# danielajisafe/A-NeRF

Hardware: AMD Instinct MI355X
Metric: rays/sec at 512×512×128 samples, 24-joint, 8×256 MLP; 1/2/4/8 GPU (higher is better)
Workload: dtype fp32-accurate split fp16: hidden and view layers after exact power-of-two scaling, x = x0+x1 and W = W0+W1 (remainders within 2^-23 of |x|, |W|), the four fp16 MFMA products x_i W_j (dropped: the remainders' ~2^-22 of |x W|, the bound of bf16x6's dropped terms), fp32 accumulate; the bone-direction a

## Files before the change

### a-nerf_amd/build.py

```python
import hashlib
import os
import subprocess
import sys
from concurrent.futures import ThreadPoolExecutor

HERE = os.path.dirname(os.path.abspath(__file__))
CSRC = os.path.join(HERE, "csrc")
HEADER = os.path.join(os.path.dirname(HERE), "include", "anerf.h")
SRC = [os.path.join(CSRC, "anerf_render.hip"), os.path.join(CSRC, "anerf_gemm.hip"),
       os.path.join(CSRC, "anerf_iso.hip"), os.path.join(CSRC, "anerf_mesh.hip"),
       os.path.join(CSRC, "anerf_raster.hip")]
SCAN_HEADER = os.path.join(CSRC, "anerf_scan.hpp")
OUT = os.path.join(HERE, "libanerf_hip.so")
STAMP = OUT + ".stamp"
OBJS = os.path.join(HERE, ".objs")
HIPCC = os.environ.get("HIPCC", "/opt/rocm/bin/hipcc")
FLAGS = ["--offload-arch=gfx950", "-O3", "-std=c++17", "-ffp-contract=off", "-fno-slp-vectorize", "-fPIC", "-shared",
         "-Wno-unused-result"]
CFLAGS = [f for f in FLAGS if f != "-shared"]


def _hash(files, extra=""):
    h = hashlib.sha256()
    h.update((" ".join(FLAGS) + extra).encode())
    for d in files:
        if os.path.isfile(d):
            h.update(os.path.basename(d).encode())
            with open(d, "rb") as f:
                h.update(f.read())
    return h.hexdigest()


def source_hash():
    deps = sorted(os.path.join(CSRC, f) for f in os.listdir(CSRC))
    deps.append(HEADER)
    return _hash(deps)


def unit_deps(src):
    name = os.path.basename(src)
    if name == "anerf_gemm.hip":
        return [src, HEADER]
    if name in ("anerf_mesh.hip", "anerf_raster.hip"):
        return [src, SCAN_HEADER, HEADER]
    if name == "anerf_iso.hip":
        return [src, os.path.join(CSRC, "anerf_iso_table.inc"), SCAN_HEADER, HEADER]
    return [src] + sorted(os.path.join(CSRC, f) for f in os.listdir(CSRC)
                          if f.endswith(".hpp") and f != os.path.basename(SCAN_HEADER)) + [HEADER]


def stamp_matches():
    if not (os.path.exists(OUT) and os.path.exists(STAMP)):
        return False
    with open(STAMP) as f:
        return f.read().strip() == source_hash()


def _object(src, verbose, force=False):
    digest = _hash(unit_deps(src), "-c")
    name = os.path.splitext(os.path.basename(src))[0]
    obj = os.path.join(OBJS, f"{name}.{digest[:20]}.o")
    if os.path.exists(obj) and not force:
        return obj
    tmp = obj + ".tmp"
    cmd = [HIPCC] + CFLAGS + ["-c", "-o", tmp, src]
    if verbose:
        print(" ".join(cmd), file=sys.stderr)
    subprocess.run(cmd, check=True)
    if _hash(unit_deps(src), "-c") != digest:
        os.remove(tmp)
        raise RuntimeError(f"sources of {name} changed during the build: the object was discarded, build again")
    for old in os.listdir(OBJS):
        if old.startswith(name + ".") and old.endswith(".o"):
            os.remove(os.path.join(OBJS, old))
    os.replace(tmp, obj)
    return obj


def build(force=False, verbose=True):
    if not force and stamp_matches():
        return OUT
    digest = source_hash()
    os.makedirs(OBJS, exist_ok=True)
    with ThreadPoolExecutor(max(1, len(SRC))) as ex:
        objs = list(ex.map(lambda s: _object(s, verbose, force), SRC))
    tmp = OUT + ".tmp"
    if os.path.exists(tmp):
        os.remove(tmp)
    cmd = [HIPCC] + FLAGS + ["-o", tmp] + objs
    if verbose:
        print(" ".join(cmd), file=sys.stderr)
    subprocess.run(cmd, check=True)
    if source_hash() != digest:
        if os.path.exists(tmp):
            os.remove(tmp)
        raise RuntimeError("sources changed during the build: the library was discarded, build again")
    os.replace(tmp, OUT)
    with open(STAMP, "w") as f:
        f.write(digest + "\n")
    return OUT


if __name__ == "__main__":
    build(force="--force" in sys.argv)
```

### a-nerf_amd/csrc/anerf_kernels.hpp

```cpp
#pragma once

template <int W, int MR, int PREC>
__device__ __forceinline__ void render_item(const ModelDev& M, const RenderArgs& A, const LdsPlan& P,
                                            float* __restrict__ lds, int64_t ray0) {
    constexpr int WH = W / 2;
    const int tid = threadIdx.x, lane = tid & 63, wave = tid >> 6;
    const int R = A.R, S = A.S, I = A.I, T = S + I;
    const int nr = (int)min((int64_t)R, A.n - ray0);

    for (int r = tid; r < nr; r += blockDim.x) {
        const int64_t i = ray0 + r;
        const float* src = A.rb + i * A.stride;
        float* d = lds + P.ray + 16 * r;
        for (int c = 0; c < 6; ++c) d[c] = src[c];
        d[6] = A.cams ? A.cams[i] : -1.0f;
        d[7] = A.near[i];
        d[8] = A.far[i];
        d[9] = norm3(src[3], src[4], src[5]);
        d[10] = __int_as_float(A.ray_pose ? A.ray_pose[i] : 0);
    }
    __syncthreads();
    for (int idx = tid; idx < nr * M.nj * 12; idx += blockDim.x) {
        const int r = idx / (M.nj * 12), e = idx % (M.nj * 12);
        const int j = e / 12, c = e % 12;
// ... 358 lines not shown
        const float px = A.pts[3 * s], py = A.pts[3 * s + 1], pz = A.pts[3 * s + 2];
        const float* dp = A.dirs + s * A.dir_stride;
        const float dx = dp[0], dy = dp[1], dz = dp[2];
        f32x16 acc[RB], h[RB];
        JointMask mask;
        Ring ring;
        int es = 0;
        const bool pre = mlp_trunk<W, MR, true, PREC>(M, net, lds + P.sk, lds + P.cut, px, py, pz, lane, lds + P.bias, uf,
                                                      wvp, acc, h, ring, mask,
                                                      PREC >= 3 ? net.wviewh : (PREC == 2 ? net.wview6 : net.wview), st,
                                                      es);
        float sig = 0.0f;
        f32x16 av[RBV];
        if constexpr (PREC >= 3) {
            const int es_h = es;
            mlp_layer_h3<RBV, RB, false, true, PREC == 4 ? 4 : 3>(av, acc, h, nullptr, net.wviewh, lane, ring, pre, nullptr,
                                                                  lds + P.bias + (M.D + 1) * W, sig, es, net.ew_view,
                                                                  M.h3_top);
            sig *= pow2f(-es_h);
        } else if constexpr (PREC == 2)
            mlp_layer_x6<RBV, RB, false, true>(av, acc, h, nullptr, net.wview6, lane, ring, pre, nullptr,
                                               lds + P.bias + (M.D + 1) * W, sig);
        else
            mlp_layer<RBV, RB, true, false, true>(av, acc, h, nullptr, net.wview, lane, ring, nullptr,
                                                  lds + P.bias + (M.D + 1) * W, sig);
        sig += __shfl_xor(sig, 32);
        sig += net.balpha;
        const float bs = PREC >= 3 ? pow2f(es) : 1.0f;
        if (M.mrv == 0) view_dir_points<RBV, 0>(av, M, net, lds + P.sk, wvp, lds + P.g, dx, dy, dz, lane, bs);
        else view_dir_points<RBV, 4>(av, M, net, lds + P.sk, wvp, lds + P.g, dx, dy, dz, lane, bs);
        float rgb[3];
#pragma unroll
        for (int c = 0; c < 3; ++c) {
            const float* wr = net.wrgb + (c * 2 + hh) * RBV * 16;
            float a = 0.0f;
#pragma unroll
            for (int rb = 0; rb < RBV; ++rb)
#pragma unroll
                for (int i = 0; i < 16; ++i) a += wr[rb * 16 + i] * relu_act(av[rb][i]);
            a += __shfl_xor(a, 32);
            if constexpr (PREC >= 3) a *= pow2f(-es);
            rgb[c] = a + net.brgb[c];
        }
        if (own && hh == 0 && s_out < A.n) {
            float* o = A.out + 4 * s_out;
            o[0] = rgb[0];
            o[1] = rgb[1];
            o[2] = rgb[2];
            o[3] = sig;
        }
    }
}

__global__ void near_far_given_kernel(const float* __restrict__ rb, int stride, int64_t n, float* __restrict__ near_out,
                                      float* __restrict__ far_out) {
    const int64_t i = (int64_t)blockIdx.x * blockDim.x + threadIdx.x;
    if (i >= n) return;
    near_out[i] = rb[i * stride + 6];
    far_out[i] = rb[i * stride + 7];
}

__global__ void near_far_kernel(const float* __restrict__ rb, int stride, int64_t n, const float* __restrict__ cyls,
                                const int32_t* __restrict__ ray_pose, int n_poses, float* __restrict__ near_out,
                                float* __restrict__ far_out, uint8_t* __restrict__ qnan) {
    const int64_t i = (int64_t)blockIdx.x * blockDim.x + threadIdx.x;
    if (i >= n) return;
    const float* r = rb + i * stride;
    const int pose = ray_pose ? ray_pose[i] : 0;
    if (pose < 0 || pose >= n_poses) {
        near_out[i] = far_out[i] = __int_as_float(0x7fc00000);
        qnan[i] = 1;
        return;
    }
    const float* cy = cyls + 5 * pose;
    const float nearv = r[6], farv = r[7];
    const float rn0 = r[0] + r[3] * nearv, rn1 = r[2] + r[5] * nearv;
    const float rf0 = r[0] + r[3] * farv, rf1 = r[2] + r[5] * farv;
    const float nc0 = cy[0] - rn0, nc1 = cy[1] - rn1;
    const float nf0 = rf0 - rn0, nf1 = rf1 - rn1;
    const float nfn = norm2(nf0, nf1);
    const float scale = norm2(r[3], r[5]);
    const float cross = nc0 * nf1 - nc1 * nf0;
    const float dist = fabsf(cross) / nfn;
    const float rad = cy[2];
    const float Q = sqrtf(rad * rad - dist * dist);
    const float K = (nc0 * nf0 + nc1 * nf1) / nfn;
    const float mask = (Q < K) ? 1.0f : 0.0f;
    near_out[i] = nearv + (mask * (K - Q)) / scale;
    far_out[i] = nearv + (K + Q) / scale;
    qnan[i] = (Q != Q) ? 1 : 0;
}

constexpr int NF_LEAVES = 1024;
constexpr int NF_LDS = 8192;

__global__ void nan_fill_kernel(const float* __restrict__ rb, int stride, int64_t n, int chunk,
                                float* __restrict__ near_io, float* __restrict__ far_io,
                                const uint8_t* __restrict__ qnan, float* __restrict__ scratch) {
    const int64_t c0 = (int64_t)blockIdx.x * chunk;
    const int64_t c1 = min(c0 + chunk, n);
    const int64_t m = c1 - c0;
    __shared__ int any, n_leaves, valid[2];
    __shared__ float means[2];
    __shared__ int leaf_off[NF_LEAVES], leaf_cnt[NF_LEAVES];
    __shared__ float leaf_sum[NF_LEAVES];
    if (threadIdx.x == 0) { any = 0; valid[0] = valid[1] = 0; }
    __syncthreads();
    for (int64_t i = c0 + threadIdx.x; i < c1; i += blockDim.x)
        if (near_io[i] != near_io[i]) any = 1;
    __syncthreads();
    if (!any) return;
    __shared__ int st_a[64], st_b[64];
    __shared__ float st_v[64];
    if (threadIdx.x == 0) n_leaves = np_pairwise_leaves(m, leaf_off, leaf_cnt, NF_LEAVES, st_a, st_b);
    __shared__ float lbuf[NF_LDS];
    float* buf = m <= NF_LDS ? lbuf : scratch + c0;
    for (int v = 0; v < 2; ++v) {
        const float* src = v == 0 ? near_io : far_io;
        int mine = 0;
        for (int64_t i = c0 + threadIdx.x; i < c1; i += blockDim.x) {
            const float x = src[i];
            buf[i - c0] = (x != x) ? 0.0f : x;
            mine += (x == x);
        }
        atomicAdd(&valid[v], mine);
        __syncthreads();
        if (n_leaves >= 0)
            for (int k = threadIdx.x; k < n_leaves; k += blockDim.x) leaf_sum[k] = np_leaf_sum(buf + leaf_off[k], leaf_cnt[k]);
        __syncthreads();
        if (threadIdx.x == 0) {
            const float sum = n_leaves >= 0 ? np_pairwise_combine(leaf_sum, m, st_a, st_b, st_v) : np_pairwise_sum(buf, m);
            means[v] = valid[v] ? (float)((double)sum / (double)valid[v]) : __int_as_float(0x7fc00000);
        }
        __syncthreads();
    }
    for (int64_t i = c0 + threadIdx.x; i < c1; i += blockDim.x) {
        if (qnan[i]) {
            const float* r = rb + i * stride;
            near_io[i] = (means[0] != means[0]) ? r[6] : means[0];
            far_io[i] = (means[1] != means[1]) ? r[7] : means[1];
        }
    }
}

struct PixelSet {
    const int64_t* idx;
    int64_t x0, y0, bw;
    __device__ __forceinline__ int64_t pixel(int64_t t, int W) const {
        return idx ? idx[t] : (y0 + t / bw) * W + x0 + t % bw;
    }
};

__global__ void gen_rays_kernel(const float* __restrict__ c2w, int H, int W, float fx, float fy, float cx, float cy,
                                PixelSet px, int64_t n, float nearv, float farv, float* __restrict__ out) {
    const int64_t t = (int64_t)blockIdx.x * blockDim.x + threadIdx.x;
    if (t >= n) return;
    const int64_t p = px.pixel(t, W);
    const float x = (float)(p % W), y = (float)(p / W);
    const float d0 = (x - cx) / fx;
    const float d1 = -(y - cy) / fy;
    const float d2 = -1.0f;
    float* o = out + t * 11;
    float dd[3];
    for (int r = 0; r < 3; ++r) {
        dd[r] = (d0 * c2w[4 * r + 0] + d1 * c2w[4 * r + 1]) + d2 * c2w[4 * r + 2];
        o[r] = c2w[4 * r + 3];
        o[3 + r] = dd[r];
    }
    o[6] = nearv;
    o[7] = farv;
    const float nn = norm3(dd[0], dd[1], dd[2]);
    o[8] = dd[0] / nn;
    o[9] = dd[1] / nn;
    o[10] = dd[2] / nn;
}

__global__ void compose_fill_kernel(const float* __restrict__ bg, int white, int64_t hw, float* __restrict__ out_rgb,
                                    float* __restrict__ out_disp, float* __restrict__ out_acc) {
    const int64_t p = (int64_t)blockIdx.x * blockDim.x + threadIdx.x;
    if (p >= hw) return;
    for (int c = 0; c < 3; ++c) out_rgb[3 * p + c] = bg ? bg[3 * p + c] : (white ? 1.0f : 0.0f);
    out_disp[p] = 0.0f;
    if (out_acc) out_acc[p] = 0.0f;
}

__global__ void compose_scatter_kernel(const float* __restrict__ rgb, const float* __restrict__ disp,
                                       const float* __restrict__ acc, PixelSet px, int W, int64_t n,
                                       float* __restrict__ out_rgb, float* __restrict__ out_disp,
                                       float* __restrict__ out_acc) {
    const int64_t i = (int64_t)blockIdx.x * blockDim.x + threadIdx.x;
    if (i >= n) return;
    const int64_t p = px.pixel(i, W);
    const float a = acc[i];
    for (int c = 0; c < 3; ++c) out_rgb[3 * p + c] = rgb[3 * i + c] + (1.0f - a) * out_rgb[3 * p + c];
    const float d = disp[i];
    out_disp[p] = (d != d) ? 0.0f : d;
    if (out_acc) out_acc[p] = a;
}

__device__ void encode_row(const ModelDev& M, const float* __restrict__ skts, float px, float py, float pz, float dx,
                           float dy, float dz, float* __restrict__ f) {
    const int nj = M.nj, nv = 1 + 2 * M.mr;
    const int cx = nj * nv + 3 * nj;
    for (int j = 0; j < nj; ++j) {
        float S[12];
        for (int r = 0; r < 3; ++r)
            for (int c = 0; c < 4; ++c) S[4 * r + c] = skts[j * 16 + 4 * r + c];
        float qx, qy, qz;
        joint_local(S, px, py, pz, qx, qy, qz);
        const float dist = norm3(qx, qy, qz);
        const float dn = fmaxf(dist, 1e-12f);
        const float w = M.use_cutoff ? cutoff_w(M.tau, dist, M.cutoff[j]) : 1.0f;
        float u, uf;
        kp_inputs(M.cut_to, M.shift_in, dist, M.cutoff[j], u, uf);
        f[j] = (M.use_cutoff && M.cutoff_inputs) ? u * w : u;
        for (int fi = 0; fi < M.mr; ++fi) {
            float s, c;
            sincosf(uf * (float)(1 << fi), &s, &c);
            f[(1 + 2 * fi) * nj + j] = s * w;
            f[(2 + 2 * fi) * nj + j] = c * w;
        }
        const float wb = M.bone_cut ? cutoff_w(M.tau_b, dist, M.cutoff_b[j]) : 1.0f;
        f[nj * nv + 3 * j + 0] = M.bone_cut ? (qx / dn) * wb : qx / dn;
        f[nj * nv + 3 * j + 1] = M.bone_cut ? (qy / dn) * wb : qy / dn;
        f[nj * nv + 3 * j + 2] = M.bone_cut ? (qz / dn) * wb : qz / dn;
        float ex, ey, ez;
        joint_rot(S, dx, dy, dz, ex, ey, ez);
        const float en = M.view_raw ? 1.0f : fmaxf(norm3(ex, ey, ez), 1e-12f);
        const float e[3] = {ex / en, ey / en, ez / en};
        const float wv = M.cutoff_viewdir ? cutoff_w(M.tau_v, dist, M.cutoff_v[j]) : 1.0f;
        for (int c = 0; c < 3; ++c) {
            f[cx + 3 * j + c] = (M.cutoff_viewdir && M.cutoff_inputs) ? e[c] * wv : e[c];
            for (int fi = 0; fi < M.mrv; ++fi) {
                float s, co;
                sincosf(e[c] * (float)(1 << fi), &s, &co);
                f[cx + (1 + 2 * fi) * 3 * nj + 3 * j + c] = s * wv;
                f[cx + (2 + 2 * fi) * 3 * nj + 3 * j + c] = co * wv;
            }
        }
    }
}

__global__ void encode_points_kernel(ModelDev M, const float* __restrict__ skts, const float* __restrict__ pts,
                                     const float* __restrict__ dirs, int64_t n, float* __restrict__ feat) {
    const int64_t i = (int64_t)blockIdx.x * blockDim.x + threadIdx.x;
    if (i >= n) return;
    const int F = M.nj * (1 + 2 * M.mr) + 3 * M.nj + 3 * M.nj * (1 + 2 * M.mrv);
    encode_row(M, skts, pts[3 * i], pts[3 * i + 1], pts[3 * i + 2], dirs[3 * i], dirs[3 * i + 1], dirs[3 * i + 2],
               feat + i * F);
}
```

### a-nerf_amd/csrc/anerf_mlp.hpp

```cpp
#pragma once

__device__ __forceinline__ __amdgpu_buffer_rsrc_t make_rsrc(const float* p) {
    return __builtin_amdgcn_make_buffer_rsrc((void*)p, 0, 0x7fffffff, 0x00020000);
}
__device__ __forceinline__ f32x2 bload2(__amdgpu_buffer_rsrc_t rs, int voff, int soff) {
    return __builtin_bit_cast(f32x2, __builtin_amdgcn_raw_buffer_load_b64(rs, voff, soff, 0));
}
__device__ __forceinline__ f32x4 bload4(__amdgpu_buffer_rsrc_t rs, int voff, int soff) {
    return __builtin_bit_cast(f32x4, __builtin_amdgcn_raw_buffer_load_b128(rs, voff, soff, 0));
}

template <int RB>
__device__ __forceinline__ void load_bias(f32x16 (&acc)[RB], const float* __restrict__ bp_lds, int hh) {
#pragma unroll
    for (int rb = 0; rb < RB; ++rb) {
        const f32x4* p = reinterpret_cast<const f32x4*>(bp_lds + (rb * 2 + hh) * 16);
        f32x4 v0 = p[0], v1 = p[1], v2 = p[2], v3 = p[3];
        acc[rb] = f32x16{v0[0], v0[1], v0[2], v0[3], v1[0], v1[1], v1[2], v1[3],
                         v2[0], v2[1], v2[2], v2[3], v3[0], v3[1], v3[2], v3[3]};
    }
}

struct Ring {
    float v[4][16];
// ... 283 lines not shown
    for (int g = 0; g < NQ; ++g) {
        __builtin_amdgcn_sched_barrier(0);
        prefetch(g);
        if constexpr (!std::is_same<Side, NoSide>::value) (*side)(g);
        const int ob = g >> 1, s = g & 1;
        out[ob] = mfma_x6(ring.v[g % 4], T[s], out[ob]);
        if (ob == 0) alpha(0, s);
        if (ob + 1 < RBI && (ob + 1 < RBO || ob == 0)) convert_half(ob + 1, s);
        if (RBI > 1) {
#pragma unroll
            for (int p = 0; p < 8; ++p)
                if (pair_group(p, QL) == (g < QL ? -1 : g) || (g == NQ - 1 && pair_group(p, QL) > g))
                    split3_block_pair(h[1], Tn, p);
        }
        x6_group_schedule();
    }
#pragma clang loop unroll(full)
    for (int ib = 1; ib < RBI; ++ib) {
        T[0] = Tn[0];
        T[1] = Tn[1];
        const bool conv_next = ib + 1 < RBI && ib + 1 >= (RBO > 2 ? RBO : 2);
        const int q0 = conv_next ? (NQ > 2 ? 2 : NQ) : 0;
#pragma clang loop unroll(full)
        for (int q = 0; q < NQ; ++q) {
            const int s = q / RBO, ob = q % RBO;
            const int g = NQ + (ib - 1) * NQ + q;
            __builtin_amdgcn_sched_barrier(0);
            prefetch(g);
            if constexpr (!std::is_same<Side, NoSide>::value) (*side)(g);
            out[ob] = mfma_x6(ring.v[g % 4], T[s], out[ob]);
            if (ob == RBO - 1) alpha(ib, s);
            if (ib + 1 < RBI) {
                if (conv_next && q < 2) convert_half(ib + 1, q);
#pragma unroll
                for (int p = 0; p < 8; ++p)
                    if (pair_group(p, q0) == q || (q == NQ - 1 && pair_group(p, q0) > q))
                        split3_block_pair(h[ib + 1], Tn, p);
            }
            x6_group_schedule();
        }
    }
}

typedef _Float16 f16x8 __attribute__((ext_vector_type(8)));
struct H3T {
    unsigned d[2][4];
    __device__ __forceinline__ f16x8 frag(int c) const {
        return __builtin_bit_cast(f16x8, u32x4{d[c][0], d[c][1], d[c][2], d[c][3]});
    }
};

__device__ __forceinline__ float pow2f(int e) { return __builtin_bit_cast(float, (e + 127) << 23); }

__device__ __forceinline__ void split2_pair(float a, float b, float t, H3T& T, int q) {
    typedef _Float16 f16x2 __attribute__((ext_vector_type(2)));
    const float xa = a * t, xb = b * t;
    const unsigned hi = __builtin_bit_cast(unsigned, __builtin_convertvector((f32x2{xa, xb}), f16x2));
    float la, lb;
    asm("v_fma_mix_f32 %0, %1, -1.0, %2 op_sel_hi:[1,0,0]" : "=v"(la) : "v"(hi), "v"(xa));
    asm("v_fma_mix_f32 %0, %1, -1.0, %2 op_sel:[1,0,0] op_sel_hi:[1,0,0]" : "=v"(lb) : "v"(hi), "v"(xb));
    T.d[0][q] = hi;
    T.d[1][q] = __builtin_bit_cast(unsigned, __builtin_convertvector((f32x2{la, lb}), f16x2));
}

__device__ __forceinline__ void split2_block_pair(const f32x16& hb, float t, H3T (&T)[2], int p) {
    const int s = p >> 2, q = p & 3;
    split2_pair(hb[8 * s + 2 * q], hb[8 * s + 2 * q + 1], t, T[s], q);
}

constexpr int H3_NLG = 2;
constexpr int H3_LEAD_IL = 4;
template <int NP, int NV = H3_IL>
__device__ __forceinline__ void h3_group_schedule() {
    group_schedule<NP, H3_NLG, 4 / H3_NLG, NV>();
}

__device__ __forceinline__ f32x16 mfma_f16_32x32x16(f16x8 a, f16x8 b, f32x16 c) {
    return __builtin_amdgcn_mfma_f32_32x32x16_f16(a, b, c, 0, 0, 0);
}

template <int NP>
__device__ __forceinline__ f32x16 mfma_h3(const float (&w)[16], int half, const H3T& x, f32x16 c) {
    const int o = 8 * half;
    const f16x8 w0 = __builtin_bit_cast(f16x8, f32x4{w[o], w[o + 1], w[o + 2], w[o + 3]});
    const f16x8 w1 = __builtin_bit_cast(f16x8, f32x4{w[o + 4], w[o + 5], w[o + 6], w[o + 7]});
    if constexpr (NP == 4) c = mfma_f16_32x32x16(w1, x.frag(1), c);
    c = mfma_f16_32x32x16(w1, x.frag(0), c);
    c = mfma_f16_32x32x16(w0, x.frag(1), c);
    return mfma_f16_32x32x16(w0, x.frag(0), c);
}

template <int RBI>
__device__ __forceinline__ float h3_scale(const f32x16 (&a)[RBI], int& es, int ew, int top, int cap = 60) {
    int m = 0;
#pragma unroll
    for (int rb = 0; rb < RBI; ++rb)
#pragma unroll
        for (int i = 0; i < 16; ++i) {
            const float v = a[rb][i];
            m = max(m, __builtin_bit_cast(int, v));
        }
    m = max(m, __shfl_xor(m, 32));
    int shift = m > 0 ? top - (m >> 23) : 0;
    shift = max(shift, -100 - es - ew);
    shift = min(shift, cap - es - ew);
    shift = min(max(shift, -126), 126);
    es += shift + ew;
    return pow2f(shift);
}

template <int RBO, int RBI, bool OUT_SAME, bool ALPHA, int NP = 3>
__device__ __forceinline__ void mlp_layer_h3(f32x16 (&out)[RBO], f32x16 (&ain)[RBI], f32x16 (&h)[RBI],
                                             const float* __restrict__ bias, const float* __restrict__ wp, int lane,
                                             Ring& ring, bool preloaded, const float* __restrict__ next,
                                             const float* __restrict__ wa, float& sig, int& es, int ew, int top,
                                             int cap = 60) {
    static_assert(RBO <= RBI, "h3 layer shape");
    constexpr int NG = 2 * RBO * RBI;
    constexpr int NS = NG / 2;
    constexpr int PS = 2;
    constexpr int NQ = 2 * RBO;
    const int hh = lane >> 5;
    const __amdgpu_buffer_rsrc_t rs = make_rsrc(wp);
    const __amdgpu_buffer_rsrc_t rn = make_rsrc(next ? next : wp);
    const float t = h3_scale<RBI>(ain, es, ew, top, cap);
    const float S = pow2f(es);
    auto convert_half = [&](int rb, int half) {
#pragma unroll
        for (int i = 8 * half; i < 8 * half + 8; ++i) h[rb][i] = relu_act(ain[rb][i]);
        if (OUT_SAME && rb < RBO) {
            const f32x4* p = reinterpret_cast<const f32x4*>(bias + (rb * 2 + hh) * 16 + 8 * half);
            const f32x4 v0 = p[0], v1 = p[1];
#pragma unroll
            for (int e = 0; e < 4; ++e) {
                out[rb][8 * half + e] = v0[e] * S;
                out[rb][8 * half + 4 + e] = v1[e] * S;
            }
        }
    };
    auto alpha = [&](int ib, int s) {
        if constexpr (ALPHA) {
            const f32x4* w4 = reinterpret_cast<const f32x4*>(wa + hh * 16 * RBI + 16 * ib + 8 * s);
            const f32x4 u0 = w4[0], u1 = w4[1];
#pragma unroll
            for (int j = 0; j < 8; ++j) sig = fmaf(j < 4 ? u0[j] : u1[j - 4], h[ib][8 * s + j], sig);
        }
    };
    if constexpr (!OUT_SAME) {
#pragma unroll
        for (int rb = 0; rb < RBO; ++rb) out[rb] = f32x16{0};
    }
    const bool has_next = next != nullptr;
    auto prefetch = [&](int g) {
        if (g & 1) return;
        const int G = g >> 1;
        if (G + PS < NS)
            load_group<16>(ring.v[(G + PS) % 4], rs, lane, G + PS);
        else if (NS % 4 == 0)
            load_group<16>(ring.v[(G + PS) % 4], rn, lane, has_next ? G + PS - NS : NS - 1);
    };
    auto pair_group = [](int p, int q0) { return q0 + (p * (NQ - q0 > 0 ? NQ - q0 : 1)) / 8; };
    if (!preloaded) {
#pragma unroll
        for (int G = 0; G < PS && G < NS; ++G) load_group<16>(ring.v[G], rs, lane, G);
    }
    convert_half(0, 0);
    convert_half(0, 1);
    H3T T[2], Tn[2];
#pragma unroll
    for (int p = 0; p < 8; ++p) split2_block_pair(h[0], t, T, p);
    constexpr int QL = NQ > 2 ? 2 : NQ;
#pragma clang loop unroll(full)
    for (int g = 0; g < NQ; ++g) {
        __builtin_amdgcn_sched_barrier(0);
        prefetch(g);
        const int ob = g >> 1, s = g & 1;
        out[ob] = mfma_h3<NP>(ring.v[(g >> 1) % 4], g & 1, T[s], out[ob]);
        if (ob == 0) alpha(0, s);
        if (ob + 1 < RBI && (ob + 1 < RBO || ob == 0)) convert_half(ob + 1, s);
        if (RBI > 1) {
#pragma unroll
            for (int p = 0; p < 8; ++p)
                if (pair_group(p, QL) == (g < QL ? -1 : g) || (g == NQ - 1 && pair_group(p, QL) > g))
                    split2_block_pair(h[1], t, Tn, p);
// ... 823 lines not shown
                if constexpr (UX6) u_part_x6<RB>(acc, M, net.wskipu6, uf, lane, ring, P == 2, xs);
            } else if (uf)
                u_part_lds<RB>(acc, M, net.wskipu, uf, lane, ring, after, xs);
            else
                u_part<RB, false>(acc, M, net.wskipu, sk, cut, px, py, pz, lane, nullptr, nullptr, nullptr, ring, after,
                                  st, xs);
            if constexpr (VX6)
                v_part_x6<RB, MR>(acc, M, net.wskipv6, sk, cut, px, py, pz, lane, mask, ring, xs);
            else
                v_part<RB, MR>(acc, M, net.wskipv, sk, cut, px, py, pz, lane, mask, st, xs);
            STAMP(st, 12);
        }
    }
    return pre6;
}

template <int W, int MR, int P>
__device__ void mlp_block(const ModelDev& M, const NetDev& net, const float* __restrict__ ray,
                          const float* __restrict__ sk, const float* __restrict__ cut, const float* __restrict__ z,
                          int n, int s0,
                          const float* __restrict__ G, float* __restrict__ raw_out, int lane,
                          unsigned long long* mfma_count, const float* __restrict__ bias, float* __restrict__ uf,
                          float* __restrict__ wvp, Stamps& st, bool store = true) {
    constexpr int RB = W / 32;
    constexpr int RBV = (W / 2) / 32;
    const int sl = lane & 31, hh = lane >> 5;
    int s = s0 + sl;
    if (s >= n) s = n - 1;
    const float zs = z[s];
    const float px = ray[0] + ray[3] * zs;
    const float py = ray[1] + ray[4] * zs;
    const float pz = ray[2] + ray[5] * zs;

    f32x16 acc[RB], h[RB];
    JointMask mask;
    Ring ring;
    int es = 0;
    const bool pre = mlp_trunk<W, MR, true, P>(M, net, sk, cut, px, py, pz, lane, bias, uf, wvp, acc, h, ring, mask,
                                               P >= 3 ? net.wviewh : (P == 2 ? net.wview6 : net.wview), st, es);
    float sig = 0.0f;
    f32x16 av[RBV];
    if constexpr (P >= 3) {
        const int es_h = es;
        mlp_layer_h3<RBV, RB, false, true, P == 4 ? 4 : 3>(av, acc, h, nullptr, net.wviewh, lane, ring, pre, nullptr,
                                           bias + (M.D + 1) * W, sig, es, net.ew_view, M.h3_top);
        sig *= pow2f(-es_h);
    } else if constexpr (P == 2)
        mlp_layer_x6<RBV, RB, false, true>(av, acc, h, nullptr, net.wview6, lane, ring, pre, nullptr,
                                           bias + (M.D + 1) * W, sig);
    else
        mlp_layer<RBV, RB, true, false, true>(av, acc, h, nullptr, net.wview, lane, ring, nullptr,
                                              bias + (M.D + 1) * W, sig);
    STAMP(st, 16);
    sig += __shfl_xor(sig, 32);
    sig += net.balpha;
    const int vsteps = view_dir_part<RBV>(av, M, G, wvp, reinterpret_cast<const unsigned*>(ray) + 12, lane,
                                          P >= 3 ? pow2f(es) : 1.0f);
    STAMP(st, 17);
    float rgb[3];
#pragma unroll
    for (int c = 0; c < 3; ++c) {
        const float* wr = net.wrgb + (c * 2 + hh) * RBV * 16;
        float a = 0.0f;
#pragma unroll
        for (int rb = 0; rb < RBV; ++rb)
#pragma unroll
            for (int i = 0; i < 16; ++i) a += wr[rb * 16 + i] * relu_act(av[rb][i]);
        a += __shfl_xor(a, 32);
        if constexpr (P >= 3) a *= pow2f(-es);
        rgb[c] = a + net.brgb[c];
    }
    STAMP(st, 13);
    if (mfma_count && lane == 0) {
        const int act = __builtin_popcountll(mask.m0) + __builtin_popcountll(mask.m1);
        const bool ux6 = (P >= 2) && (RB % 4 == 0) && uf != nullptr;
        constexpr bool vx6 = (P >= 2) && (RB % 4 == 0);
        const int npe = (P >= 3 && ux6 && M.enc16) ? (P == 4 ? 4 : 3) : 6;
        const int xk = (ux6 ? 0 : 3 * M.njh2) + (vx6 ? 0 : act * VPart<MR>::KB);
        long long k = (long long)xk * RB + (long long)vsteps * RBV;
        const int nx = (M.skip + 1 < M.D) ? 2 : 1;
        if (ux6) atomicAdd(mfma_count + 1, (unsigned long long)(nx * ((3 * M.njh2 + 7) / 8) * RB * npe));
        if (vx6) atomicAdd(mfma_count + 1, (unsigned long long)(nx * act * VPartX6<MR, 1>::KS * RB * npe));
        constexpr int NPR = P == 2 ? 6 : (P == 4 ? 4 : 3);
        if (P >= 2)
            atomicAdd(mfma_count + 1, (unsigned long long)(RBV * RB * 2 * NPR));
        else
            k += (long long)(W / 2) * RBV;
        if (M.skip + 1 < M.D) k += (long long)xk * RB;
        const long long hid = (long long)(M.D - 1) * RB * RB;
        if (P != 0) {
            atomicAdd(mfma_count + 1, (unsigned long long)(hid * 2 * NPR));
        } else {
            k += hid * 16;
        }
        atomicAdd(mfma_count, (unsigned long long)k);
    }
    if (store && hh == 0 && s0 + sl < n) {
        float* o = raw_out + 4 * (s0 + sl);
        o[0] = rgb[0];
        o[1] = rgb[1];
        o[2] = rgb[2];
        o[3] = sig;
    }
}
```

### a-nerf_amd/csrc/anerf_render.hip

```cpp
#include <hip/hip_runtime.h>

#include <algorithm>
#include <cmath>
#include <cstdio>
#include <cstdlib>
#include <cstring>
#include <string>
#include <type_traits>
#include <vector>

#include "../../include/anerf.h"
#include "anerf_device.hpp"

using namespace anerf;

#include "anerf_types.hpp"
#include "anerf_mlp.hpp"
#include "anerf_stages.hpp"
#include "anerf_kernels.hpp"
#include "anerf_train.hpp"
#include "anerf_trainfwd.hpp"
#include "anerf_pose.hpp"
#include "anerf_boxes.hpp"
#include "anerf_batch.hpp"
#include "anerf_pack.hpp"


int anerf_internal_fail(int code, const char* msg) { return fail(code, msg); }

#ifdef ANERF_STAMPS
static unsigned long long* g_stamps = nullptr;
extern "C" void anerf_diag_set_stamps(unsigned long long* p) { g_stamps = p; }
#endif

namespace {
struct TfLayout {
    size_t wx0, wl[MAXL], wskipx, wf, wvf, wvv, wvc, total;
};
size_t tf_regs_floats(int n_out, int n_in) { return (size_t)2 * (n_out / 32) * (n_in / 32) * 768; }
size_t tf_mem_floats(int n_out, int K) { return (size_t)tf_xsteps(K) * (n_out / 32) * 768; }
int tf_check(const anerf_mlp_shape* s) {
    if (!s) return fail(ANERF_EINVAL, "anerf_mlp_forward: NULL shape");
    if (s->width != 128 && s->width != 256)
        return fail(ANERF_EINVAL, "anerf_mlp_forward: width 128 or 256");
    if (s->depth < 1 || s->depth > MAXL) return fail(ANERF_EINVAL, "anerf_mlp_forward: depth 1..16");
    if (s->dnet < 1 || s->dnet % 4 || s->nv < 1 || s->nv % 4 || s->cfc < 0 || s->cfc % 4)
        return fail(ANERF_EINVAL, "anerf_mlp_forward: dnet, nv, cfc must be multiples of 4");
    return ANERF_OK;
}
TfLayout tf_layout(const anerf_mlp_shape* s) {
    const int W = s->width, D = s->depth;
    TfLayout L = {};
    size_t o = 0;
    L.wx0 = o; o += tf_mem_floats(W, s->dnet);
    for (int i = 1; i < D; ++i) { L.wl[i] = o; o += tf_regs_floats(W, W); }
    const bool has_skip = s->skip >= 0 && s->skip + 1 < D;
    L.wskipx = o; if (has_skip) o += tf_mem_floats(W, s->dnet);
    L.wf = o; o += tf_regs_floats(W, W);
    L.wvf = o; o += tf_regs_floats(W / 2, W);
    L.wvv = o; o += tf_mem_floats(W / 2, s->nv);
    L.wvc = o; if (s->cfc > 0) o += tf_mem_floats(W / 2, s->cfc);
    L.total = o;
    return L;
}
template <int W>
hipError_t tf_launch(const TfArgs& a, long long m, hipStream_t st) {
    constexpr int RB = W / 32;
    const size_t lds = sizeof(float) * ((size_t)(a.D + 1) * W + W / 2 + 2 * RB * 16 + 3 * 2 * (RB / 2) * 16 +
                                        (size_t)4 * 32 * (W + 4));
    const hipError_t attr = hipFuncSetAttribute((const void*)train_mlp_fwd_kernel<W>,
                                                hipFuncAttributeMaxDynamicSharedMemorySize, 160 * 1024);
    if (attr != hipSuccess) return attr;
// ... 1051 lines not shown
```

Measured before the change: 1.193 million.

## Compile split-fp16 kernels in separate unit with MFMA VGPR form and permlane reductions

```diff
diff --git a/a-nerf_amd/build.py b/a-nerf_amd/build.py
--- a/a-nerf_amd/build.py
+++ b/a-nerf_amd/build.py
@@ -7,7 +7,8 @@
 HERE = os.path.dirname(os.path.abspath(__file__))
 CSRC = os.path.join(HERE, "csrc")
 HEADER = os.path.join(os.path.dirname(HERE), "include", "anerf.h")
-SRC = [os.path.join(CSRC, "anerf_render.hip"), os.path.join(CSRC, "anerf_gemm.hip"),
+SRC = [os.path.join(CSRC, "anerf_render.hip"), os.path.join(CSRC, "anerf_render_f16.hip"),
+       os.path.join(CSRC, "anerf_gemm.hip"),
        os.path.join(CSRC, "anerf_iso.hip"), os.path.join(CSRC, "anerf_mesh.hip"),
        os.path.join(CSRC, "anerf_raster.hip")]
 SCAN_HEADER = os.path.join(CSRC, "anerf_scan.hpp")
@@ -18,11 +19,16 @@
 FLAGS = ["--offload-arch=gfx950", "-O3", "-std=c++17", "-ffp-contract=off", "-fno-slp-vectorize", "-fPIC", "-shared",
          "-Wno-unused-result"]
 CFLAGS = [f for f in FLAGS if f != "-shared"]
+RENDER_F16_FLAGS = ["-mllvm", "-amdgpu-mfma-vgpr-form"]
+UNIT_FLAGS = {"anerf_render_f16.hip": RENDER_F16_FLAGS}
 
 
 def _hash(files, extra=""):
     h = hashlib.sha256()
     h.update((" ".join(FLAGS) + extra).encode())
+    for name in sorted(UNIT_FLAGS):
+        if any(os.path.basename(d) == name for d in files):
+            h.update((name + " " + " ".join(UNIT_FLAGS[name])).encode())
     for d in files:
         if os.path.isfile(d):
             h.update(os.path.basename(d).encode())
@@ -63,7 +69,7 @@
     if os.path.exists(obj) and not force:
         return obj
     tmp = obj + ".tmp"
-    cmd = [HIPCC] + CFLAGS + ["-c", "-o", tmp, src]
+    cmd = [HIPCC] + CFLAGS + UNIT_FLAGS.get(os.path.basename(src), []) + ["-c", "-o", tmp, src]
     if verbose:
         print(" ".join(cmd), file=sys.stderr)
     subprocess.run(cmd, check=True)
diff --git a/a-nerf_amd/csrc/anerf_kernels.hpp b/a-nerf_amd/csrc/anerf_kernels.hpp
--- a/a-nerf_amd/csrc/anerf_kernels.hpp
+++ b/a-nerf_amd/csrc/anerf_kernels.hpp
@@ -434,200 +434,17 @@
     }
 }
 
-__global__ void near_far_given_kernel(const float* __restrict__ rb, int stride, int64_t n, float* __restrict__ near_out,
-                                      float* __restrict__ far_out) {
-    const int64_t i = (int64_t)blockIdx.x * blockDim.x + threadIdx.x;
-    if (i >= n) return;
-    near_out[i] = rb[i * stride + 6];
-    far_out[i] = rb[i * stride + 7];
-}
-
-__global__ void near_far_kernel(const float* __restrict__ rb, int stride, int64_t n, const float* __restrict__ cyls,
-                                const int32_t* __restrict__ ray_pose, int n_poses, float* __restrict__ near_out,
-                                float* __restrict__ far_out, uint8_t* __restrict__ qnan) {
-    const int64_t i = (int64_t)blockIdx.x * blockDim.x + threadIdx.x;
-    if (i >= n) return;
-    const float* r = rb + i * stride;
-    const int pose = ray_pose ? ray_pose[i] : 0;
-    if (pose < 0 || pose >= n_poses) {
-        near_out[i] = far_out[i] = __int_as_float(0x7fc00000);
-        qnan[i] = 1;
-        return;
-    }
-    const float* cy = cyls + 5 * pose;
-    const float nearv = r[6], farv = r[7];
-    const float rn0 = r[0] + r[3] * nearv, rn1 = r[2] + r[5] * nearv;
-    const float rf0 = r[0] + r[3] * farv, rf1 = r[2] + r[5] * farv;
-    const float nc0 = cy[0] - rn0, nc1 = cy[1] - rn1;
-    const float nf0 = rf0 - rn0, nf1 = rf1 - rn1;
-    const float nfn = norm2(nf0, nf1);
-    const float scale = norm2(r[3], r[5]);
-    const float cross = nc0 * nf1 - nc1 * nf0;
-    const float dist = fabsf(cross) / nfn;
-    const float rad = cy[2];
-    const float Q = sqrtf(rad * rad - dist * dist);
-    const float K = (nc0 * nf0 + nc1 * nf1) / nfn;
-    const float mask = (Q < K) ? 1.0f : 0.0f;
-    near_out[i] = nearv + (mask * (K - Q)) / scale;
-    far_out[i] = nearv + (K + Q) / scale;
-    qnan[i] = (Q != Q) ? 1 : 0;
-}
-
-constexpr int NF_LEAVES = 1024;
-constexpr int NF_LDS = 8192;
-
-__global__ void nan_fill_kernel(const float* __restrict__ rb, int stride, int64_t n, int chunk,
-                                float* __restrict__ near_io, float* __restrict__ far_io,
-                                const uint8_t* __restrict__ qnan, float* __restrict__ scratch) {
-    const int64_t c0 = (int64_t)blockIdx.x * chunk;
-    const int64_t c1 = min(c0 + chunk, n);
-    const int64_t m = c1 - c0;
-    __shared__ int any, n_leaves, valid[2];
-    __shared__ float means[2];
-    __shared__ int leaf_off[NF_LEAVES], leaf_cnt[NF_LEAVES];
-    __shared__ float leaf_sum[NF_LEAVES];
-    if (threadIdx.x == 0) { any = 0; valid[0] = valid[1] = 0; }
-    __syncthreads();
-    for (int64_t i = c0 + threadIdx.x; i < c1; i += blockDim.x)
-        if (near_io[i] != near_io[i]) any = 1;
-    __syncthreads();
-    if (!any) return;
-    __shared__ int st_a[64], st_b[64];
-    __shared__ float st_v[64];
-    if (threadIdx.x == 0) n_leaves = np_pairwise_leaves(m, leaf_off, leaf_cnt, NF_LEAVES, st_a, st_b);
-    __shared__ float lbuf[NF_LDS];
-    float* buf = m <= NF_LDS ? lbuf : scratch + c0;
-    for (int v = 0; v < 2; ++v) {
-        const float* src = v == 0 ? near_io : far_io;
-        int mine = 0;
-        for (int64_t i = c0 + threadIdx.x; i < c1; i += blockDim.x) {
-            const float x = src[i];
-            buf[i - c0] = (x != x) ? 0.0f : x;
-            mine += (x == x);
-        }
-        atomicAdd(&valid[v], mine);
-        __syncthreads();
-        if (n_leaves >= 0)
-            for (int k = threadIdx.x; k < n_leaves; k += blockDim.x) leaf_sum[k] = np_leaf_sum(buf + leaf_off[k], leaf_cnt[k]);
-        __syncthreads();
-        if (threadIdx.x == 0) {
-            const float sum = n_leaves >= 0 ? np_pairwise_combine(leaf_sum, m, st_a, st_b, st_v) : np_pairwise_sum(buf, m);
-            means[v] = valid[v] ? (float)((double)sum / (double)valid[v]) : __int_as_float(0x7fc00000);
-        }
-        __syncthreads();
-    }
-    for (int64_t i = c0 + threadIdx.x; i < c1; i += blockDim.x) {
-        if (qnan[i]) {
-            const float* r = rb + i * stride;
-            near_io[i] = (means[0] != means[0]) ? r[6] : means[0];
-            far_io[i] = (means[1] != means[1]) ? r[7] : means[1];
-        }
-    }
-}
-
-struct PixelSet {
-    const int64_t* idx;
-    int64_t x0, y0, bw;
-    __device__ __forceinline__ int64_t pixel(int64_t t, int W) const {
-        return idx ? idx[t] : (y0 + t / bw) * W + x0 + t % bw;
-    }
-};
-
-__global__ void gen_rays_kernel(const float* __restrict__ c2w, int H, int W, float fx, float fy, float cx, float cy,
-                                PixelSet px, int64_t n, float nearv, float farv, float* __restrict__ out) {
-    const int64_t t = (int64_t)blockIdx.x * blockDim.x + threadIdx.x;
-    if (t >= n) return;
-    const int64_t p = px.pixel(t, W);
-    const float x = (float)(p % W), y = (float)(p / W);
-    const float d0 = (x - cx) / fx;
-    const float d1 = -(y - cy) / fy;
-    const float d2 = -1.0f;
-    float* o = out + t * 11;
-    float dd[3];
-    for (int r = 0; r < 3; ++r) {
-        dd[r] = (d0 * c2w[4 * r + 0] + d1 * c2w[4 * r + 1]) + d2 * c2w[4 * r + 2];
-        o[r] = c2w[4 * r + 3];
-        o[3 + r] = dd[r];
-    }
-    o[6] = nearv;
-    o[7] = farv;
-    const float nn = norm3(dd[0], dd[1], dd[2]);
-    o[8] = dd[0] / nn;
-    o[9] = dd[1] / nn;
-    o[10] = dd[2] / nn;
-}
-
-__global__ void compose_fill_kernel(const float* __restrict__ bg, int white, int64_t hw, float* __restrict__ out_rgb,
-                                    float* __restrict__ out_disp, float* __restrict__ out_acc) {
-    const int64_t p = (int64_t)blockIdx.x * blockDim.x + threadIdx.x;
-    if (p >= hw) return;
-    for (int c = 0; c < 3; ++c) out_rgb[3 * p + c] = bg ? bg[3 * p + c] : (white ? 1.0f : 0.0f);
-    out_disp[p] = 0.0f;
-    if (out_acc) out_acc[p] = 0.0f;
-}
-
-__global__ void compose_scatter_kernel(const float* __restrict__ rgb, const float* __restrict__ disp,
-                                       const float* __restrict__ acc, PixelSet px, int W, int64_t n,
-                                       float* __restrict__ out_rgb, float* __restrict__ out_disp,
-                                       float* __restrict__ out_acc) {
-    const int64_t i = (int64_t)blockIdx.x * blockDim.x + threadIdx.x;
-    if (i >= n) return;
-    const int64_t p = px.pixel(i, W);
-    const float a = acc[i];
-    for (int c = 0; c < 3; ++c) out_rgb[3 * p + c] = rgb[3 * i + c] + (1.0f - a) * out_rgb[3 * p + c];
-    const float d = disp[i];
-    out_disp[p] = (d != d) ? 0.0f : d;
-    if (out_acc) out_acc[p] = a;
-}
-
-__device__ void encode_row(const ModelDev& M, const float* __restrict__ skts, float px, float py, float pz, float dx,
-                           float dy, float dz, float* __restrict__ f) {
-    const int nj = M.nj, nv = 1 + 2 * M.mr;
-    const int cx = nj * nv + 3 * nj;
-    for (int j = 0; j < nj; ++j) {
-        float S[12];
-        for (int r = 0; r < 3; ++r)
-            for (int c = 0; c < 4; ++c) S[4 * r + c] = skts[j * 16 + 4 * r + c];
-        float qx, qy, qz;
-        joint_local(S, px, py, pz, qx, qy, qz);
-        const float dist = norm3(qx, qy, qz);
-        const float dn = fmaxf(dist, 1e-12f);
-        const float w = M.use_cutoff ? cutoff_w(M.tau, dist, M.cutoff[j]) : 1.0f;
-        float u, uf;
-        kp_inputs(M.cut_to, M.shift_in, dist, M.cutoff[j], u, uf);
-        f[j] = (M.use_cutoff && M.cutoff_inputs) ? u * w : u;
-        for (int fi = 0; fi < M.mr; ++fi) {
-            float s, c;
-            sincosf(uf * (float)(1 << fi), &s, &c);
-            f[(1 + 2 * fi) * nj + j] = s * w;
-            f[(2 + 2 * fi) * nj + j] = c * w;
-        }
-        const float wb = M.bone_cut ? cutoff_w(M.tau_b, dist, M.cutoff_b[j]) : 1.0f;
-        f[nj * nv + 3 * j + 0] = M.bone_cut ? (qx / dn) * wb : qx / dn;
-        f[nj * nv + 3 * j + 1] = M.bone_cut ? (qy / dn) * wb : qy / dn;
-        f[nj * nv + 3 * j + 2] = M.bone_cut ? (qz / dn) * wb : qz / dn;
-        float ex, ey, ez;
-        joint_rot(S, dx, dy, dz, ex, ey, ez);
-        const float en = M.view_raw ? 1.0f : fmaxf(norm3(ex, ey, ez), 1e-12f);
-        const float e[3] = {ex / en, ey / en, ez / en};
-        const float wv = M.cutoff_viewdir ? cutoff_w(M.tau_v, dist, M.cutoff_v[j]) : 1.0f;
-        for (int c = 0; c < 3; ++c) {
-            f[cx + 3 * j + c] = (M.cutoff_viewdir && M.cutoff_inputs) ? e[c] * wv : e[c];
-            for (int fi = 0; fi < M.mrv; ++fi) {
-                float s, co;
-                sincosf(e[c] * (float)(1 << fi), &s, &co);
-                f[cx + (1 + 2 * fi) * 3 * nj + 3 * j + c] = s * wv;
-                f[cx + (2 + 2 * fi) * 3 * nj + 3 * j + c] = co * wv;
-            }
-        }
-    }
-}
-
-__global__ void encode_points_kernel(ModelDev M, const float* __restrict__ skts, const float* __restrict__ pts,
-                                     const float* __restrict__ dirs, int64_t n, float* __restrict__ feat) {
-    const int64_t i = (int64_t)blockIdx.x * blockDim.x + threadIdx.x;
-    if (i >= n) return;
-    const int F = M.nj * (1 + 2 * M.mr) + 3 * M.nj + 3 * M.nj * (1 + 2 * M.mrv);
-    encode_row(M, skts, pts[3 * i], pts[3 * i + 1], pts[3 * i + 2], dirs[3 * i], dirs[3 * i + 1], dirs[3 * i + 2],
-               feat + i * F);
-}
+#define ANERF_F16_KERNEL(KW, K, ARGS, WW, MM)                              \
+    KW template __global__ void K<WW, MM, 3>(ModelDev, ARGS, LdsPlan);    \
+    KW template __global__ void K<WW, MM, 4>(ModelDev, ARGS, LdsPlan);
+#ifdef ANERF_AB_FAST
+#define ANERF_F16_SHAPES(KW, K, ARGS) ANERF_F16_KERNEL(KW, K, ARGS, 256, 7)
+#else
+#define ANERF_F16_SHAPES(KW, K, ARGS)                                                                     \
+    ANERF_F16_KERNEL(KW, K, ARGS, 256, 7) ANERF_F16_KERNEL(KW, K, ARGS, 128, 7) ANERF_F16_KERNEL(KW, K, ARGS, 64, 7) \
+    ANERF_F16_KERNEL(KW, K, ARGS, 256, 10) ANERF_F16_KERNEL(KW, K, ARGS, 128, 10) ANERF_F16_KERNEL(KW, K, ARGS, 64, 10)
+#endif
+#define ANERF_F16_INSTANCES(KW)                       \
+    ANERF_F16_SHAPES(KW, render_kernel, RenderArgs)   \
+    ANERF_F16_SHAPES(KW, density_kernel, DensityArgs) \
+    ANERF_F16_SHAPES(KW, radiance_kernel, RadianceArgs)
diff --git a/a-nerf_amd/csrc/anerf_kernels_small.hpp b/a-nerf_amd/csrc/anerf_kernels_small.hpp
--- /dev/null
+++ b/a-nerf_amd/csrc/anerf_kernels_small.hpp
@@ -0,0 +1,199 @@
+#pragma once
+
+__global__ void near_far_given_kernel(const float* __restrict__ rb, int stride, int64_t n, float* __restrict__ near_out,
+                                      float* __restrict__ far_out) {
+    const int64_t i = (int64_t)blockIdx.x * blockDim.x + threadIdx.x;
+    if (i >= n) return;
+    near_out[i] = rb[i * stride + 6];
+    far_out[i] = rb[i * stride + 7];
+}
+
+__global__ void near_far_kernel(const float* __restrict__ rb, int stride, int64_t n, const float* __restrict__ cyls,
+                                const int32_t* __restrict__ ray_pose, int n_poses, float* __restrict__ near_out,
+                                float* __restrict__ far_out, uint8_t* __restrict__ qnan) {
+    const int64_t i = (int64_t)blockIdx.x * blockDim.x + threadIdx.x;
+    if (i >= n) return;
+    const float* r = rb + i * stride;
+    const int pose = ray_pose ? ray_pose[i] : 0;
+    if (pose < 0 || pose >= n_poses) {
+        near_out[i] = far_out[i] = __int_as_float(0x7fc00000);
+        qnan[i] = 1;
+        return;
+    }
+    const float* cy = cyls + 5 * pose;
+    const float nearv = r[6], farv = r[7];
+    const float rn0 = r[0] + r[3] * nearv, rn1 = r[2] + r[5] * nearv;
+    const float rf0 = r[0] + r[3] * farv, rf1 = r[2] + r[5] * farv;
+    const float nc0 = cy[0] - rn0, nc1 = cy[1] - rn1;
+    const float nf0 = rf0 - rn0, nf1 = rf1 - rn1;
+    const float nfn = norm2(nf0, nf1);
+    const float scale = norm2(r[3], r[5]);
+    const float cross = nc0 * nf1 - nc1 * nf0;
+    const float dist = fabsf(cross) / nfn;
+    const float rad = cy[2];
+    const float Q = sqrtf(rad * rad - dist * dist);
+    const float K = (nc0 * nf0 + nc1 * nf1) / nfn;
+    const float mask = (Q < K) ? 1.0f : 0.0f;
+    near_out[i] = nearv + (mask * (K - Q)) / scale;
+    far_out[i] = nearv + (K + Q) / scale;
+    qnan[i] = (Q != Q) ? 1 : 0;
+}
+
+constexpr int NF_LEAVES = 1024;
+constexpr int NF_LDS = 8192;
+
+__global__ void nan_fill_kernel(const float* __restrict__ rb, int stride, int64_t n, int chunk,
+                                float* __restrict__ near_io, float* __restrict__ far_io,
+                                const uint8_t* __restrict__ qnan, float* __restrict__ scratch) {
+    const int64_t c0 = (int64_t)blockIdx.x * chunk;
+    const int64_t c1 = min(c0 + chunk, n);
+    const int64_t m = c1 - c0;
+    __shared__ int any, n_leaves, valid[2];
+    __shared__ float means[2];
+    __shared__ int leaf_off[NF_LEAVES], leaf_cnt[NF_LEAVES];
+    __shared__ float leaf_sum[NF_LEAVES];
+    if (threadIdx.x == 0) { any = 0; valid[0] = valid[1] = 0; }
+    __syncthreads();
+    for (int64_t i = c0 + threadIdx.x; i < c1; i += blockDim.x)
+        if (near_io[i] != near_io[i]) any = 1;
+    __syncthreads();
+    if (!any) return;
+    __shared__ int st_a[64], st_b[64];
+    __shared__ float st_v[64];
+    if (threadIdx.x == 0) n_leaves = np_pairwise_leaves(m, leaf_off, leaf_cnt, NF_LEAVES, st_a, st_b);
+    __shared__ float lbuf[NF_LDS];
+    float* buf = m <= NF_LDS ? lbuf : scratch + c0;
+    for (int v = 0; v < 2; ++v) {
+        const float* src = v == 0 ? near_io : far_io;
+        int mine = 0;
+        for (int64_t i = c0 + threadIdx.x; i < c1; i += blockDim.x) {
+            const float x = src[i];
+            buf[i - c0] = (x != x) ? 0.0f : x;
+            mine += (x == x);
+        }
+        atomicAdd(&valid[v], mine);
+        __syncthreads();
+        if (n_leaves >= 0)
+            for (int k = threadIdx.x; k < n_leaves; k += blockDim.x) leaf_sum[k] = np_leaf_sum(buf + leaf_off[k], leaf_cnt[k]);
+        __syncthreads();
+        if (threadIdx.x == 0) {
+            const float sum = n_leaves >= 0 ? np_pairwise_combine(leaf_sum, m, st_a, st_b, st_v) : np_pairwise_sum(buf, m);
+            means[v] = valid[v] ? (float)((double)sum / (double)valid[v]) : __int_as_float(0x7fc00000);
+        }
+        __syncthreads();
+    }
+    for (int64_t i = c0 + threadIdx.x; i < c1; i += blockDim.x) {
+        if (qnan[i]) {
+            const float* r = rb + i * stride;
+            near_io[i] = (means[0] != means[0]) ? r[6] : means[0];
+            far_io[i] = (means[1] != means[1]) ? r[7] : means[1];
+        }
+    }
+}
+
+struct PixelSet {
+    const int64_t* idx;
+    int64_t x0, y0, bw;
+    __device__ __forceinline__ int64_t pixel(int64_t t, int W) const {
+        return idx ? idx[t] : (y0 + t / bw) * W + x0 + t % bw;
+    }
+};
+
+__global__ void gen_rays_kernel(const float* __restrict__ c2w, int H, int W, float fx, float fy, float cx, float cy,
+                                PixelSet px, int64_t n, float nearv, float farv, float* __restrict__ out) {
+    const int64_t t = (int64_t)blockIdx.x * blockDim.x + threadIdx.x;
+    if (t >= n) return;
+    const int64_t p = px.pixel(t, W);
+    const float x = (float)(p % W), y = (float)(p / W);
+    const float d0 = (x - cx) / fx;
+    const float d1 = -(y - cy) / fy;
+    const float d2 = -1.0f;
+    float* o = out + t * 11;
+    float dd[3];
+    for (int r = 0; r < 3; ++r) {
+        dd[r] = (d0 * c2w[4 * r + 0] + d1 * c2w[4 * r + 1]) + d2 * c2w[4 * r + 2];
+        o[r] = c2w[4 * r + 3];
+        o[3 + r] = dd[r];
+    }
+    o[6] = nearv;
+    o[7] = farv;
+    const float nn = norm3(dd[0], dd[1], dd[2]);
+    o[8] = dd[0] / nn;
+    o[9] = dd[1] / nn;
+    o[10] = dd[2] / nn;
+}
+
+__global__ void compose_fill_kernel(const float* __restrict__ bg, int white, int64_t hw, float* __restrict__ out_rgb,
+                                    float* __restrict__ out_disp, float* __restrict__ out_acc) {
+    const int64_t p = (int64_t)blockIdx.x * blockDim.x + threadIdx.x;
+    if (p >= hw) return;
+    for (int c = 0; c < 3; ++c) out_rgb[3 * p + c] = bg ? bg[3 * p + c] : (white ? 1.0f : 0.0f);
+    out_disp[p] = 0.0f;
+    if (out_acc) out_acc[p] = 0.0f;
+}
+
+__global__ void compose_scatter_kernel(const float* __restrict__ rgb, const float* __restrict__ disp,
+                                       const float* __restrict__ acc, PixelSet px, int W, int64_t n,
+                                       float* __restrict__ out_rgb, float* __restrict__ out_disp,
+                                       float* __restrict__ out_acc) {
+    const int64_t i = (int64_t)blockIdx.x * blockDim.x + threadIdx.x;
+    if (i >= n) return;
+    const int64_t p = px.pixel(i, W);
+    const float a = acc[i];
+    for (int c = 0; c < 3; ++c) out_rgb[3 * p + c] = rgb[3 * i + c] + (1.0f - a) * out_rgb[3 * p + c];
+    const float d = disp[i];
+    out_disp[p] = (d != d) ? 0.0f : d;
+    if (out_acc) out_acc[p] = a;
+}
+
+__device__ void encode_row(const ModelDev& M, const float* __restrict__ skts, float px, float py, float pz, float dx,
+                           float dy, float dz, float* __restrict__ f) {
+    const int nj = M.nj, nv = 1 + 2 * M.mr;
+    const int cx = nj * nv + 3 * nj;
+    for (int j = 0; j < nj; ++j) {
+        float S[12];
+        for (int r = 0; r < 3; ++r)
+            for (int c = 0; c < 4; ++c) S[4 * r + c] = skts[j * 16 + 4 * r + c];
+        float qx, qy, qz;
+        joint_local(S, px, py, pz, qx, qy, qz);
+        const float dist = norm3(qx, qy, qz);
+        const float dn = fmaxf(dist, 1e-12f);
+        const float w = M.use_cutoff ? cutoff_w(M.tau, dist, M.cutoff[j]) : 1.0f;
+        float u, uf;
+        kp_inputs(M.cut_to, M.shift_in, dist, M.cutoff[j], u, uf);
+        f[j] = (M.use_cutoff && M.cutoff_inputs) ? u * w : u;
+        for (int fi = 0; fi < M.mr; ++fi) {
+            float s, c;
+            sincosf(uf * (float)(1 << fi), &s, &c);
+            f[(1 + 2 * fi) * nj + j] = s * w;
+            f[(2 + 2 * fi) * nj + j] = c * w;
+        }
+        const float wb = M.bone_cut ? cutoff_w(M.tau_b, dist, M.cutoff_b[j]) : 1.0f;
+        f[nj * nv + 3 * j + 0] = M.bone_cut ? (qx / dn) * wb : qx / dn;
+        f[nj * nv + 3 * j + 1] = M.bone_cut ? (qy / dn) * wb : qy / dn;
+        f[nj * nv + 3 * j + 2] = M.bone_cut ? (qz / dn) * wb : qz / dn;
+        float ex, ey, ez;
+        joint_rot(S, dx, dy, dz, ex, ey, ez);
+        const float en = M.view_raw ? 1.0f : fmaxf(norm3(ex, ey, ez), 1e-12f);
+        const float e[3] = {ex / en, ey / en, ez / en};
+        const float wv = M.cutoff_viewdir ? cutoff_w(M.tau_v, dist, M.cutoff_v[j]) : 1.0f;
+        for (int c = 0; c < 3; ++c) {
+            f[cx + 3 * j + c] = (M.cutoff_viewdir && M.cutoff_inputs) ? e[c] * wv : e[c];
+            for (int fi = 0; fi < M.mrv; ++fi) {
+                float s, co;
+                sincosf(e[c] * (float)(1 << fi), &s, &co);
+                f[cx + (1 + 2 * fi) * 3 * nj + 3 * j + c] = s * wv;
+                f[cx + (2 + 2 * fi) * 3 * nj + 3 * j + c] = co * wv;
+            }
+        }
+    }
+}
+
+__global__ void encode_points_kernel(ModelDev M, const float* __restrict__ skts, const float* __restrict__ pts,
+                                     const float* __restrict__ dirs, int64_t n, float* __restrict__ feat) {
+    const int64_t i = (int64_t)blockIdx.x * blockDim.x + threadIdx.x;
+    if (i >= n) return;
+    const int F = M.nj * (1 + 2 * M.mr) + 3 * M.nj + 3 * M.nj * (1 + 2 * M.mrv);
+    encode_row(M, skts, pts[3 * i], pts[3 * i + 1], pts[3 * i + 2], dirs[3 * i], dirs[3 * i + 1], dirs[3 * i + 2],
+               feat + i * F);
+}
diff --git a/a-nerf_amd/csrc/anerf_mlp.hpp b/a-nerf_amd/csrc/anerf_mlp.hpp
--- a/a-nerf_amd/csrc/anerf_mlp.hpp
+++ b/a-nerf_amd/csrc/anerf_mlp.hpp
@@ -359,6 +359,17 @@
 
 __device__ __forceinline__ float pow2f(int e) { return __builtin_bit_cast(float, (e + 127) << 23); }
 
+__device__ __forceinline__ int max_halves(int x) {
+    const auto r = __builtin_amdgcn_permlane32_swap((unsigned)x, (unsigned)x, false, false);
+    return max((int)r[0], (int)r[1]);
+}
+__device__ __forceinline__ float sum_halves(float x) {
+    const unsigned u = __builtin_bit_cast(unsigned, x);
+    const auto r = __builtin_amdgcn_permlane32_swap(u, u, false, false);
+    const unsigned lo = r[0], hi = r[1];
+    return __builtin_bit_cast(float, lo) + __builtin_bit_cast(float, hi);
+}
+
 __device__ __forceinline__ void split2_pair(float a, float b, float t, H3T& T, int q) {
     typedef _Float16 f16x2 __attribute__((ext_vector_type(2)));
     const float xa = a * t, xb = b * t;
@@ -407,7 +418,7 @@
             const float v = a[rb][i];
             m = max(m, __builtin_bit_cast(int, v));
         }
-    m = max(m, __shfl_xor(m, 32));
+    m = max_halves(m);
     int shift = m > 0 ? top - (m >> 23) : 0;
     shift = max(shift, -100 - es - ew);
     shift = min(shift, cap - es - ew);
@@ -432,11 +443,13 @@
     const __amdgpu_buffer_rsrc_t rn = make_rsrc(next ? next : wp);
     const float t = h3_scale<RBI>(ain, es, ew, top, cap);
     const float S = pow2f(es);
+    int hb = 0;
+    if constexpr (OUT_SAME) asm volatile("v_mbcnt_lo_u32_b32 %0, %1, 0" : "=v"(hb) : "s"(0x80000000u));
     auto convert_half = [&](int rb, int half) {
 #pragma unroll
         for (int i = 8 * half; i < 8 * half + 8; ++i) h[rb][i] = relu_act(ain[rb][i]);
         if (OUT_SAME && rb < RBO) {
-            const f32x4* p = reinterpret_cast<const f32x4*>(bias + (rb * 2 + hh) * 16 + 8 * half);
+            const f32x4* p = reinterpret_cast<const f32x4*>(bias + (rb * 2 + hb) * 16 + 8 * half);
             const f32x4 v0 = p[0], v1 = p[1];
 #pragma unroll
             for (int e = 0; e < 4; ++e) {
@@ -1366,7 +1379,8 @@
         mlp_layer<RBV, RB, true, false, true>(av, acc, h, nullptr, net.wview, lane, ring, nullptr,
                                               bias + (M.D + 1) * W, sig);
     STAMP(st, 16);
-    sig += __shfl_xor(sig, 32);
+    if constexpr (P >= 3) sig = sum_halves(sig);
+    else sig += __shfl_xor(sig, 32);
     sig += net.balpha;
     const int vsteps = view_dir_part<RBV>(av, M, G, wvp, reinterpret_cast<const unsigned*>(ray) + 12, lane,
                                           P >= 3 ? pow2f(es) : 1.0f);
@@ -1380,7 +1394,8 @@
         for (int rb = 0; rb < RBV; ++rb)
 #pragma unroll
             for (int i = 0; i < 16; ++i) a += wr[rb * 16 + i] * relu_act(av[rb][i]);
-        a += __shfl_xor(a, 32);
+        if constexpr (P >= 3) a = sum_halves(a);
+        else a += __shfl_xor(a, 32);
         if constexpr (P >= 3) a *= pow2f(-es);
         rgb[c] = a + net.brgb[c];
     }
diff --git a/a-nerf_amd/csrc/anerf_render.hip b/a-nerf_amd/csrc/anerf_render.hip
--- a/a-nerf_amd/csrc/anerf_render.hip
+++ b/a-nerf_amd/csrc/anerf_render.hip
@@ -18,6 +18,8 @@
 #include "anerf_mlp.hpp"
 #include "anerf_stages.hpp"
 #include "anerf_kernels.hpp"
+ANERF_F16_INSTANCES(extern)
+#include "anerf_kernels_small.hpp"
 #include "anerf_train.hpp"
 #include "anerf_trainfwd.hpp"
 #include "anerf_pose.hpp"
diff --git a/a-nerf_amd/csrc/anerf_render_f16.hip b/a-nerf_amd/csrc/anerf_render_f16.hip
--- /dev/null
+++ b/a-nerf_amd/csrc/anerf_render_f16.hip
@@ -0,0 +1,18 @@
+#include <hip/hip_runtime.h>
+
+#include <algorithm>
+#include <cmath>
+#include <cstring>
+#include <type_traits>
+
+#include "../../include/anerf.h"
+#include "anerf_device.hpp"
+
+using namespace anerf;
+
+#include "anerf_types.hpp"
+#include "anerf_mlp.hpp"
+#include "anerf_stages.hpp"
+#include "anerf_kernels.hpp"
+
+ANERF_F16_INSTANCES()
```

New measurement: 1.205 million (median of 6 runs). +1.0%, better.
